# riffusion/riffusion-hobby

Measured on AMD Instinct MI355X. Metric: spectrogram_tiles_per_sec_griffinlim32, higher is better.
Workload: dtype f32

## Files before the change

riffusion-hobby_amd/csrc/rfx_imel.hip:

```cpp
#include <hip/hip_runtime.h>

#include "rfx_core.h"
#include "rfx_kernels.h"
#include <stdlib.h>

namespace rfx {

constexpr int kImelThreads = 256;

template <int BPT>
__global__ void __launch_bounds__(kImelThreads) imel_kernel(ImelArgs a) {
  extern __shared__ __attribute__((aligned(16))) char smem[];
  const ImelTables& tb = a.tb;
  const int nb = tb.f_hi - tb.f_lo;
  float* spec_s = reinterpret_cast<float*>(smem);
  float* w_s = spec_s + ((nb + 3) & ~3);
  float* diff_s = w_s + ((tb.nnz + 3) & ~3);
  float* red_s = diff_s + ((a.M + 1 + 3) & ~3);
  float* hist_s = red_s + 4;

  const int frame = blockIdx.x;
  const int b = frame / a.T, t = frame - b * a.T;
  const int clip = b / a.C;
  const int tid = threadIdx.x;
// ... 160 lines not shown
    for (int p4 = tid; p4 < (a.out_stride >> 2); p4 += nthr) {
      const int4 b = pb4[p4];
      out4[p4] = float4{value_at(b.x), value_at(b.y), value_at(b.z), value_at(b.w)};
    }
  } else {
    for (int p = tid; p < a.out_stride; p += nthr) out[p] = value_at(tb.pos_bin[p]);
  }
}

constexpr float kImelScale = 8.673617379884035e-19f;
constexpr float kImelUnscale = 1152921504606846976.0f;
__device__ __forceinline__ void imel_set_scale(ImelArgs& a, int clip) {
  a.sc = a.clip_scale ? a.clip_scale[2 * clip] : kImelScale;
  a.un = a.clip_scale ? a.clip_scale[2 * clip + 1] : kImelUnscale;
}
#ifndef RFX_IMEL_CLAMP
#define RFX_IMEL_CLAMP 1
#endif
#ifndef RFX_IMEL_UFORM
#define RFX_IMEL_UFORM 1
#endif

__device__ __forceinline__ float clamp_step(float x) {
#if RFX_IMEL_CLAMP
  return __builtin_amdgcn_fmed3f(x, 0.f, 1.f);
#else
  return fmaxf(0.f, x);
#endif
}

#ifndef RFX_IMEL_PK
#define RFX_IMEL_PK 1
#endif
#if RFX_IMEL_PK
using c2 = float __attribute__((ext_vector_type(2)));
__device__ __forceinline__ c2 bc2(float x) { return c2{x, x}; }
__device__ __forceinline__ c2 pk_step_clamp(c2 spec, unsigned long long nl2, c2 buf) {
#if RFX_IMEL_CLAMP
  asm("v_pk_fma_f32 %0, %1, %2, %0 clamp" : "+v"(spec) : "s"(nl2), "v"(buf));
  return spec;
#else
  const float nl = __builtin_bit_cast(float, (unsigned)nl2);
  const c2 r = __builtin_elementwise_fma(bc2(nl), buf, spec);
  return c2{fmaxf(0.f, r.x), fmaxf(0.f, r.y)};
#endif
}

template <int N, bool UF>
struct GroupState {
  static constexpr int NP = (N + 1) / 2;
  c2 spec[NP], buf[NP], w0[NP], w1[NP];
  int f0, n;
};

template <int N, bool UF>
__device__ __forceinline__ void group_load(GroupState<N, UF>& g, int grp, const ImelArgs& a, int frame, unsigned rbase, float scale) {
  const ImelTables& tb = a.tb;
  g.f0 = grp >= 0 ? tb.grp_start[grp] : 0;
  g.n = grp >= 0 ? tb.grp_start[grp + 1] - g.f0 : 0;
#pragma unroll
  for (int i = 0; i < 2 * g.NP; ++i) {
    const bool ok = i < g.n;
    const int f = g.f0 + (ok ? i : 0);
    const float w0 = ok ? tb.bin_w0[f] : 0.f, w1 = ok ? tb.bin_w1[f] : 0.f;
    const float sp = ok ? scale * (a.spec0 ? a.spec0[(size_t)frame * a.n_stft + f] : rand_unit(rbase, f)) : 0.f;
    if (i & 1) { g.w0[i >> 1].y = w0; g.w1[i >> 1].y = w1; g.spec[i >> 1].y = sp; g.buf[i >> 1].y = 0.f; }
    else       { g.w0[i >> 1].x = w0; g.w1[i >> 1].x = w1; g.spec[i >> 1].x = sp; g.buf[i >> 1].x = 0.f; }
  }
}
template <int N, bool UF>
__device__ __forceinline__ void group_ab(const GroupState<N, UF>& g, float& A, float& B) {
  c2 sa = bc2(0.f), sb = bc2(0.f);
#pragma unroll
  for (int i = 0; i < g.NP; ++i) {
    sa = __builtin_elementwise_fma(g.w0[i], g.spec[i], sa);
    sb = __builtin_elementwise_fma(g.w1[i], g.spec[i], sb);
  }
  A = sa.x + sa.y;
  B = sb.x + sb.y;
}
template <int N, bool UF>
__device__ __forceinline__ void group_step(GroupState<N, UF>& g, float d0, float d1, float mom, unsigned long long nl2) {
  const c2 vm = bc2(mom), v0 = bc2(d0), v1 = bc2(d1), vd = bc2(d0 - d1);
#pragma unroll
  for (int i = 0; i < g.NP; ++i) {
    c2 bnew;
    if (UF) {
      bnew = __builtin_elementwise_fma(vm, g.buf[i], v1);
      bnew = __builtin_elementwise_fma(vd, g.w0[i], bnew);
    } else {
      bnew = vm * g.buf[i];
      bnew = __builtin_elementwise_fma(v0, g.w0[i], bnew);
      bnew = __builtin_elementwise_fma(v1, g.w1[i], bnew);
    }
    g.buf[i] = bnew;
  }
#pragma unroll
  for (int i = 0; i < g.NP; ++i) g.spec[i] = pk_step_clamp(g.spec[i], nl2, g.buf[i]);
}
template <int N, bool UF>
__device__ __forceinline__ void group_stage(const GroupState<N, UF>& g, const ImelTables& tb, float* stage, float unscale) {
#pragma unroll
  for (int i = 0; i < 2 * g.NP; ++i)
    if (i < g.n) stage[g.f0 + i - tb.f_lo] = unscale * ((i & 1) ? g.spec[i >> 1].y : g.spec[i >> 1].x);
}
#else
template <int N, bool UF>
struct GroupState {
  float spec[N], buf[N], w0[N], w1[N];
  int f0, n;
};

template <int N, bool UF>
__device__ __forceinline__ void group_load(GroupState<N, UF>& g, int grp, const ImelArgs& a, int frame, unsigned rbase, float scale) {
  const ImelTables& tb = a.tb;
  g.f0 = grp >= 0 ? tb.grp_start[grp] : 0;
  g.n = grp >= 0 ? tb.grp_start[grp + 1] - g.f0 : 0;
#pragma unroll
  for (int i = 0; i < N; ++i) {
    const bool ok = i < g.n;
    const int f = g.f0 + (ok ? i : 0);
    g.w0[i] = ok ? tb.bin_w0[f] : 0.f;
    g.w1[i] = ok ? tb.bin_w1[f] : 0.f;
    g.spec[i] = ok ? scale * (a.spec0 ? a.spec0[(size_t)frame * a.n_stft + f] : rand_unit(rbase, f)) : 0.f;
    g.buf[i] = 0.f;
  }
}
template <int N, bool UF>
__device__ __forceinline__ void group_ab(const GroupState<N, UF>& g, float& A, float& B) {
  float a0 = 0.f, a1 = 0.f, b0 = 0.f, b1 = 0.f;
#pragma unroll
  for (int i = 0; i < N; i += 2) {
    a0 = fmaf(g.w0[i], g.spec[i], a0);
    b0 = fmaf(g.w1[i], g.spec[i], b0);
    if (i + 1 < N) {
      a1 = fmaf(g.w0[i + 1], g.spec[i + 1], a1);
      b1 = fmaf(g.w1[i + 1], g.spec[i + 1], b1);
    }
  }
  A = a0 + a1;
  B = b0 + b1;
}
template <int N, bool UF>
__device__ __forceinline__ void group_step(GroupState<N, UF>& g, float d0, float d1, float mom, unsigned long long nl2) {
  const float lrg = -__builtin_bit_cast(float, (unsigned)nl2);
  const float dd = d0 - d1;
#pragma unroll
  for (int i = 0; i < N; ++i) {
    float bnew;
    if (UF) {
      bnew = fmaf(mom, g.buf[i], d1);
      bnew = fmaf(dd, g.w0[i], bnew);
    } else {
      bnew = mom * g.buf[i];
      bnew = fmaf(d0, g.w0[i], bnew);
      bnew = fmaf(d1, g.w1[i], bnew);
    }
    g.buf[i] = bnew;
    g.spec[i] = clamp_step(fmaf(-lrg, bnew, g.spec[i]));
  }
}
template <int N, bool UF>
__device__ __forceinline__ void group_stage(const GroupState<N, UF>& g, const ImelTables& tb, float* stage, float unscale) {
#pragma unroll
  for (int i = 0; i < N; ++i)
    if (i < g.n) stage[g.f0 + i - tb.f_lo] = unscale * g.spec[i];
}

#endif

template <int NLO, int NHI, bool UF>
__device__ __forceinline__ void imel_group_body(ImelArgs a, char* smem, int tid, int frame, bool live) {
  const ImelTables& tb = a.tb;
  const int M = a.M;
  float* Ab = reinterpret_cast<float*>(smem);
  float* Bb = Ab + 2 * (M + 4);
  float* part = Bb + 2 * (M + 4);

  const int b = frame / a.T, t = frame - b * a.T;
  const int clip = b / a.C;
  const int steps = a.it_limit ? a.it_limit[clip] : a.max_iter;
  if (a.it_limit && steps >= a.max_iter) return;
  const unsigned rbase = rand_frame_key(a.seed, a.frame_base + (unsigned long long)frame);
  imel_set_scale(a, clip);

  const int gH = (M - 1 - tid >= 0) ? M - 1 - tid : -1;
  const int gL = (tid < M - kImelThreads) ? tid : -1;
  const float kScale = RFX_IMEL_CLAMP ? a.sc : 1.f, kUnscale = RFX_IMEL_CLAMP ? a.un : 1.f;
  GroupState<NLO, false> lo;
  GroupState<NHI, UF> hi;
  group_load(lo, gL, a, frame, rbase, kScale);
  group_load(hi, gH, a, frame, rbase, kScale);
  auto melat = [&](int m) { return (m >= 0 && m < M) ? kScale * a.mel[((size_t)b * M + m) * a.T + t] : 0.f; };
  const float mL0 = gL >= 0 ? melat(gL) : 0.f, mL1 = gL >= 0 ? melat(gL + 1) : 0.f;
  const float mH0 = gH >= 0 ? melat(gH) : 0.f, mH1 = gH >= 0 ? melat(gH + 1) : 0.f;
  for (int i = tid; i < 4 * (M + 4); i += kImelThreads) Ab[i] = 0.f;
  const float lrg = a.lr * (-2.0f / (float)(a.C * a.T));
  const unsigned nlb = __builtin_amdgcn_readfirstlane(__builtin_bit_cast(unsigned, -lrg));
  const unsigned long long nl2 = ((unsigned long long)nlb << 32) | nlb;
  const int xL = (gL >= 0 ? gL : M + 1) + 1, xH = (gH >= 0 ? gH : M + 1) + 1;
  const bool noH1 = UF && gH == M - 1;
  const int wave = tid >> 6;
  __syncthreads();

  auto sgd_step = [&](int it, float* __restrict__ Ap, float* __restrict__ Bp) {
    float AL, BL, AH, BH;
    group_ab(lo, AL, BL);
    group_ab(hi, AH, BH);
    Ap[xL] = AL; Bp[xL] = BL;
    Ap[xH] = AH; Bp[xH] = BH;
    __syncthreads();
    const float bLm = Bp[xL - 1], aLp = Ap[xL + 1], bHm = Bp[xH - 1], aHp = Ap[xH + 1];
    const float dL0 = mL0 - AL - bLm;
    const float dL1 = mL1 - aLp - BL;
    const float dH0 = mH0 - AH - bHm;
    const float dH1 = noH1 ? 0.f : mH1 - aHp - BH;
#ifndef RFX_ABL_IMEL_NO_LOSS
    const float uL = kUnscale * dL0, uH = kUnscale * dH0;
    const float sq = wave_sum(fmaf(uL, uL, uH * uH));
    if ((tid & 63) == 0) part[4 * it + wave] = sq;
#endif
    group_step(lo, dL0, dL1, a.momentum, nl2);
    group_step(hi, dH0, dH1, a.momentum, nl2);
  };
  float* const A0 = Ab, * const A1 = Ab + (M + 4), * const B0 = Bb, * const B1 = Bb + (M + 4);
  int it = 0;
  for (; it + 1 < steps; it += 2) {
    sgd_step(it, A0, B0);
    sgd_step(it + 1, A1, B1);
  }
  if (it < steps) sgd_step(it, A0, B0);
  __syncthreads();

  float* stage = reinterpret_cast<float*>(smem + imel_group_lds_bytes(M, a.max_iter));
  group_stage(lo, tb, stage, kUnscale);
  group_stage(hi, tb, stage, kUnscale);
  __syncthreads();
  if (!live) return;
  imel_emit_frame(a, stage, frame, rbase, tid, kImelThreads);
  if (a.loss_hist && !a.it_limit)
    for (int i = tid; i < a.max_iter; i += kImelThreads)
      a.loss_hist[(size_t)frame * a.max_iter + i] = i < steps ? (part[4 * i] + part[4 * i + 1]) + (part[4 * i + 2] + part[4 * i + 3]) : 0.f;
}

template <int NLO, int NHI>
__global__ void __launch_bounds__(kImelThreads) imel_group_kernel(ImelArgs a) {
  extern __shared__ __attribute__((aligned(16))) char smem[];
  imel_group_body<NLO, NHI, false>(a, smem, threadIdx.x, blockIdx.x, true);
}
#ifndef RFX_IMEL_WAVES_PER_EU
#define RFX_IMEL_WAVES_PER_EU 4
#endif
#ifndef RFX_IMEL_WAVES_PER_EU_UF
#define RFX_IMEL_WAVES_PER_EU_UF 4
#endif
#ifndef RFX_IMEL_FPW
#define RFX_IMEL_FPW 1
#endif

template <int FPW, int WPE, bool UF, int L0, int H0, int L1, int H1, int L2, int H2, int L3, int H3>
__global__ void __launch_bounds__(kImelThreads * FPW) __attribute__((amdgpu_waves_per_eu(WPE)))
imel_group_kernel_perwave(ImelArgs a) {
  extern __shared__ __attribute__((aligned(16))) char smem[];
  const int wave = __builtin_amdgcn_readfirstlane(threadIdx.x >> 6);
  const int slot = wave >> 2, w4 = wave & 3;
  const int cls = FPW == 1 ? w4 : FPW == 2 ? (slot ? 3 - w4 : w4) : ((w4 + slot) & 3);
  const int tid = cls * 64 + (threadIdx.x & 63);
  const int nframes = a.B * a.T;
  int frame = blockIdx.x * FPW + slot;
  const bool live = frame < nframes;
  if (!live) frame = nframes - 1;
  char* my = smem + (size_t)slot * imel_frame_lds_bytes(a.M, a.max_iter, a.tb.f_hi - a.tb.f_lo);
  switch (cls) {
    case 0: imel_group_body<L0, H0, UF>(a, my, tid, frame, live); break;
    case 1: imel_group_body<L1, H1, UF>(a, my, tid, frame, live); break;
    case 2: imel_group_body<L2, H2, UF>(a, my, tid, frame, live); break;
    default: imel_group_body<L3, H3, UF>(a, my, tid, frame, live); break;
  }
}


#if RFX_IMEL_PK
constexpr int kDppWaveShl1 = 0x130, kDppWaveShr1 = 0x138;
template <int CTRL>
__device__ __forceinline__ float wave_shift(float old, float src) {
  return __builtin_bit_cast(float, __builtin_amdgcn_update_dpp(__builtin_bit_cast(int, old), __builtin_bit_cast(int, src), CTRL, 0xf, 0xf, false));
}
__device__ __forceinline__ c2 pk_add_clamp(c2 x, c2 v) {
  asm("v_pk_add_f32 %0, %0, %1 clamp" : "+v"(x) : "v"(v));
  return x;
}
__device__ __forceinline__ c2 pk_fma_clamp(c2 x, c2 v, c2 m) {
  asm("v_pk_fma_f32 %0, %1, %2, %0 clamp" : "+v"(x) : "v"(v), "v"(m));
  return x;
}

__device__ __forceinline__ void fma_in_place(float& x, unsigned m_sgpr, float c) { asm("v_fma_f32 %0, %1, %0, %2" : "+v"(x) : "s"(m_sgpr), "v"(c)); }

template <int NP, int NF, bool UF>
struct WvChunk {
  static constexpr int NT = NP - NF;
  c2 spec[NP];
  c2 mask[NT > 0 ? NT : 1];
  float a0, s0, a1, s1;
  float m0;
  float C, G;
};

template <int NP, int NF, bool UF>
__device__ __forceinline__ void wv_load(WvChunk<NP, NF, UF>& k, int g, const ImelArgs& a, int frame, int b, int t, unsigned rbase) {
  const ImelTables& tb = a.tb;
  const int f0 = tb.grp_start[g], n = tb.grp_start[g + 1] - f0;
  k.a0 = tb.lin[g];
  k.s0 = tb.lin[a.M + g];
  k.a1 = tb.lin[2 * a.M + g];
  k.s1 = tb.lin[3 * a.M + g];
  k.m0 = a.sc * a.mel[((size_t)b * a.M + g) * a.T + t];
  k.C = 0.f;
  k.G = 0.f;
#pragma unroll
  for (int i = 0; i < 2 * NP; ++i) {
    const bool ok = i < n;
    const int f = f0 + (ok ? i : 0);
    const float sp = ok ? a.sc * (a.spec0 ? a.spec0[(size_t)frame * a.n_stft + f] : rand_unit(rbase, f)) : 0.f;
    if (i & 1) k.spec[i >> 1].y = sp; else k.spec[i >> 1].x = sp;
    if (i >= 2 * NF) {
      if (i & 1) k.mask[(i >> 1) - NF].y = ok ? 1.f : 0.f; else k.mask[(i >> 1) - NF].x = ok ? 1.f : 0.f;
    }
  }
}
template <int NPA, int NFA, int NPB, int NFB, bool UFA, bool UFB>
__device__ __forceinline__ void wv_sums2(const WvChunk<NPA, NFA, UFA>& ka, const WvChunk<NPB, NFB, UFB>& kb, c2& SA, c2& QA, c2& SB, c2& QB) {
  static_assert(NPA >= 2 && NPB >= 2, "every chunk holds at least two pairs");
  SA = ka.spec[0] + ka.spec[1];
  SB = kb.spec[0] + kb.spec[1];
  QA = ka.spec[1];
  QB = kb.spec[1];
#pragma unroll
  for (int p = 2; p < (NPA > NPB ? NPA : NPB); ++p) {
    if (p < NPA) SA = SA + ka.spec[p];
    if (p < NPB) SB = SB + kb.spec[p];
    if (p < NPA) QA = __builtin_elementwise_fma(bc2((float)p), ka.spec[p], QA);
    if (p < NPB) QB = __builtin_elementwise_fma(bc2((float)p), kb.spec[p], QB);
  }
}
template <int NP, int NF, bool UF>
__device__ __forceinline__ void wv_update(WvChunk<NP, NF, UF>& k, float vx, float vy, float w2) {
  const c2 base = c2{vx, vy}, s2 = bc2(w2);
  c2 v[NP];
  v[0] = base;
#pragma unroll
  for (int p = 1; p < NP; ++p) v[p] = __builtin_elementwise_fma(bc2((float)p), s2, base);
#pragma unroll
  for (int p = 0; p < NP; ++p) k.spec[p] = p < NF ? pk_add_clamp(k.spec[p], v[p]) : pk_fma_clamp(k.spec[p], v[p], k.mask[p < NF ? 0 : p - NF]);
}
template <int NP, int NF, bool UF>
__device__ __forceinline__ void wv_stage(const WvChunk<NP, NF, UF>& k, int g, const ImelTables& tb, float* stage, float unscale) {
  const int f0 = tb.grp_start[g], n = tb.grp_start[g + 1] - f0;
#pragma unroll
  for (int i = 0; i < 2 * NP; ++i)
    if (i < n) stage[f0 + i - tb.f_lo] = unscale * ((i & 1) ? k.spec[i >> 1].y : k.spec[i >> 1].x);
}

template <int NP, bool UF>
struct LineGroup {
  c2 spec[NP], mask[NP];
  float a0, s0, a1, s1;
  float C, G;
};
template <int NP, bool UF>
__device__ __forceinline__ void line_load(LineGroup<NP, UF>& k, int g, const ImelArgs& a, int frame, unsigned rbase) {
  const ImelTables& tb = a.tb;
  const int f0 = g >= 0 ? tb.grp_start[g] : 0, n = g >= 0 ? tb.grp_start[g + 1] - f0 : 0;
  k.a0 = g >= 0 ? tb.lin[g] : 0.f;
  k.s0 = g >= 0 ? tb.lin[a.M + g] : 0.f;
  k.a1 = g >= 0 ? tb.lin[2 * a.M + g] : 0.f;
  k.s1 = g >= 0 ? tb.lin[3 * a.M + g] : 0.f;
  k.C = 0.f;
  k.G = 0.f;
#pragma unroll
  for (int i = 0; i < 2 * NP; ++i) {
    const bool ok = i < n;
    const int f = f0 + (ok ? i : 0);
    const float sp = ok ? a.sc * (a.spec0 ? a.spec0[(size_t)frame * a.n_stft + f] : rand_unit(rbase, f)) : 0.f;
    if (i & 1) { k.spec[i >> 1].y = sp; k.mask[i >> 1].y = ok ? 1.f : 0.f; }
    else       { k.spec[i >> 1].x = sp; k.mask[i >> 1].x = ok ? 1.f : 0.f; }
  }
}
template <int NP, bool UF>
__device__ __forceinline__ void line_ab(const LineGroup<NP, UF>& k, float& A, float& B) {
  static_assert(NP >= 2, "a line group holds at least two pairs");
  c2 Sa = k.spec[0], Sb = k.spec[1], Qa = bc2(0.f), Qb = k.spec[1];
#pragma unroll
  for (int p = 2; p < NP; ++p) {
    if (p & 1) { Sb = Sb + k.spec[p]; Qb = __builtin_elementwise_fma(bc2((float)p), k.spec[p], Qb); }
    else       { Sa = Sa + k.spec[p]; Qa = __builtin_elementwise_fma(bc2((float)p), k.spec[p], Qa); }
  }
  const c2 S = Sa + Sb, Q = Qa + Qb;
  const float s = S.x + S.y, h = Q.x + Q.y;
  const float q = fmaf(2.f, h, S.y);
  A = fmaf(k.s0, q, k.a0 * s);
  B = UF ? s - A : fmaf(k.s1, q, k.a1 * s);
}
template <int NP, bool UF>
__device__ __forceinline__ void line_step(LineGroup<NP, UF>& k, float n0, float n1, float mom) {
  float cc, st;
  if (UF) {
    const float dd = n0 - n1;
    cc = fmaf(dd, k.a0, n1);
    st = dd * k.s0;
  } else {
    cc = fmaf(n1, k.a1, n0 * k.a0);
    st = fmaf(n1, k.s1, n0 * k.s0);
  }
  k.C = fmaf(mom, k.C, cc);
  k.G = fmaf(mom, k.G, st);
  const c2 base = c2{k.C, k.C + k.G}, s2 = bc2(k.G + k.G);
#pragma unroll
  for (int p = 0; p < NP; ++p) {
    const c2 v = p == 0 ? base : __builtin_elementwise_fma(bc2((float)p), s2, base);
    k.spec[p] = pk_fma_clamp(k.spec[p], v, k.mask[p]);
  }
}
template <int NP, bool UF>
__device__ __forceinline__ void line_stage(const LineGroup<NP, UF>& k, int g, const ImelTables& tb, float* stage, float unscale) {
  if (g < 0) return;
  const int f0 = tb.grp_start[g], n = tb.grp_start[g + 1] - f0;
#pragma unroll
  for (int i = 0; i < 2 * NP; ++i)
    if (i < n) stage[f0 + i - tb.f_lo] = unscale * ((i & 1) ? k.spec[i >> 1].y : k.spec[i >> 1].x);
}

template <int NLO, int NHI, bool UF>
__device__ __forceinline__ void imel_line_body(ImelArgs a, char* smem, int tid, int frame) {
  const ImelTables& tb = a.tb;
  const int M = a.M;
  float* Ab = reinterpret_cast<float*>(smem);
  float* Bb = Ab + 2 * (M + 4);
  float* part = Bb + 2 * (M + 4);
  const int b = frame / a.T, t = frame - b * a.T;
  const int clip = b / a.C;
  const int steps = a.it_limit ? a.it_limit[clip] : a.max_iter;
  if (a.it_limit && steps >= a.max_iter) return;
  const unsigned rbase = rand_frame_key(a.seed, a.frame_base + (unsigned long long)frame);
  imel_set_scale(a, clip);
  int gH = (M - 1 - tid >= 0) ? M - 1 - tid : -1;
  int gL = (tid < M - kImelThreads) ? tid : -1;
  if (gH >= 0 && gH < tb.line_from) {
    gL = gH;
    gH = -1;
  }
  GroupState<NLO, false> lo;
  LineGroup<(NHI + 1) / 2, UF> hi;
  group_load(lo, gL, a, frame, rbase, a.sc);
  line_load(hi, gH, a, frame, rbase);
  auto melat = [&](int m) { return (m >= 0 && m < M) ? a.sc * a.mel[((size_t)b * M + m) * a.T + t] : 0.f; };
  const float mL0 = gL >= 0 ? melat(gL) : 0.f, mL1 = gL >= 0 ? melat(gL + 1) : 0.f;
  const float mH0 = gH >= 0 ? melat(gH) : 0.f, mH1 = gH >= 0 ? melat(gH + 1) : 0.f;
  for (int i = tid; i < 4 * (M + 4); i += kImelThreads) Ab[i] = 0.f;
  const float lrg = a.lr * (-2.0f / (float)(a.C * a.T));
  const float nl = -lrg;
  const unsigned nlb = __builtin_amdgcn_readfirstlane(__builtin_bit_cast(unsigned, nl));
  const unsigned long long nl2 = ((unsigned long long)nlb << 32) | nlb;
  const int xL = (gL >= 0 ? gL : M + 1) + 1, xH = (gH >= 0 ? gH : M + 1) + 1;
  const bool noH1 = UF && gH == M - 1;
  const int wave = tid >> 6;
  __syncthreads();

  auto sgd_step = [&](int it, float* __restrict__ Ap, float* __restrict__ Bp) {
    float AL, BL, AH, BH;
    group_ab(lo, AL, BL);
    line_ab(hi, AH, BH);
    Ap[xL] = AL; Bp[xL] = BL;
    Ap[xH] = AH; Bp[xH] = BH;
    __syncthreads();
    const float bLm = Bp[xL - 1], aLp = Ap[xL + 1], bHm = Bp[xH - 1], aHp = Ap[xH + 1];
    const float dL0 = mL0 - AL - bLm;
    const float dL1 = mL1 - aLp - BL;
    const float dH0 = mH0 - AH - bHm;
    const float dH1 = noH1 ? 0.f : mH1 - aHp - BH;
    const float uL = a.un * dL0, uH = a.un * dH0;
    const float sq = wave_sum(fmaf(uL, uL, uH * uH));
    if ((tid & 63) == 0) part[4 * it + wave] = sq;
    group_step(lo, dL0, dL1, a.momentum, nl2);
    line_step(hi, nl * dH0, nl * dH1, a.momentum);
  };
  float* const A0 = Ab, * const A1 = Ab + (M + 4), * const B0 = Bb, * const B1 = Bb + (M + 4);
  int it = 0;
  for (; it + 1 < steps; it += 2) {
    sgd_step(it, A0, B0);
    sgd_step(it + 1, A1, B1);
  }
  if (it < steps) sgd_step(it, A0, B0);
  __syncthreads();

  float* stage = reinterpret_cast<float*>(smem + imel_group_lds_bytes(M, a.max_iter));
  group_stage(lo, tb, stage, a.un);
  line_stage(hi, gH, tb, stage, a.un);
  __syncthreads();
  imel_emit_frame(a, stage, frame, rbase, tid, kImelThreads);
  if (a.loss_hist && !a.it_limit)
    for (int i = tid; i < a.max_iter; i += kImelThreads)
      a.loss_hist[(size_t)frame * a.max_iter + i] = i < steps ? (part[4 * i] + part[4 * i + 1]) + (part[4 * i + 2] + part[4 * i + 3]) : 0.f;
}

template <bool UF, int L0, int H0, int L1, int H1, int L2, int H2, int L3, int H3>
__global__ void __launch_bounds__(kImelThreads) __attribute__((amdgpu_waves_per_eu(2, 2))) imel_line_kernel_perwave(ImelArgs a) {
  extern __shared__ __attribute__((aligned(16))) char smem[];
  const int cls = __builtin_amdgcn_readfirstlane(threadIdx.x >> 6);
  const int tid = threadIdx.x;
  const int frame = blockIdx.x;
  switch (cls) {
    case 0: imel_line_body<L0, H0, UF>(a, smem, tid, frame); break;
    case 1: imel_line_body<L1, H1, UF>(a, smem, tid, frame); break;
    case 2: imel_line_body<L2, H2, UF>(a, smem, tid, frame); break;
    default: imel_line_body<L3, H3, UF>(a, smem, tid, frame); break;
  }
}

#define RFX_WV_CHUNKS(X) X(0) X(1) X(2) X(3) X(4) X(5) X(6) X(7)
#define RFX_WV_LO(X) X(0) X(1) X(2) X(3)
#define RFX_WV_HI(X) X(4) X(5) X(6) X(7)

template <bool UFH>
__global__ void __launch_bounds__(64) __attribute__((amdgpu_waves_per_eu(2, 2))) imel_wave_kernel(ImelArgs a) {
  extern __shared__ __attribute__((aligned(16))) char smem[];
  float* part = reinterpret_cast<float*>(smem);
  const ImelTables& tb = a.tb;
  const int lane = threadIdx.x, frame = blockIdx.x;
  const int b = frame / a.T, t = frame - b * a.T;
  const int clip = b / a.C;
  const int steps = a.it_limit ? a.it_limit[clip] : a.max_iter;
  if (a.it_limit && steps >= a.max_iter) return;
  const unsigned rbase = rand_frame_key(a.seed, a.frame_base + (unsigned long long)frame);
  imel_set_scale(a, clip);
  for (int i = lane; i < a.max_iter; i += 64) part[i] = 0.f;
  const unsigned part_lds = (unsigned)(size_t)(__attribute__((address_space(3))) char*)smem;

#define RFX_WV_DECL(c, UF) WvChunk<kImelWavePairs[c], kImelWaveFullPairs[c], UF> k##c;
  RFX_WV_DECL(0, false) RFX_WV_DECL(1, false) RFX_WV_DECL(2, false) RFX_WV_DECL(3, false)
  RFX_WV_DECL(4, UFH) RFX_WV_DECL(5, UFH) RFX_WV_DECL(6, UFH) RFX_WV_DECL(7, UFH)
#undef RFX_WV_DECL
#define RFX_WV_LOAD(c) wv_load(k##c, imel_wave_group(c, lane), a, frame, b, t, rbase);
  RFX_WV_CHUNKS(RFX_WV_LOAD)
#undef RFX_WV_LOAD

  const float nl = -(a.lr * (-2.0f / (float)(a.C * a.T)));
  const unsigned mom_s = __builtin_amdgcn_readfirstlane(__builtin_bit_cast(unsigned, a.momentum));
  __builtin_amdgcn_s_waitcnt(0xc07f);

  for (int it = 0; it < steps; ++it) {
    float A0, A1, A2, A3, A4, A5, A6, A7, B0, B1, B2, B3, B4, B5, B6, B7;
    {
      c2 S0, Q0, S1, Q1, S2, Q2, S3, Q3;
      wv_sums2(k0, k1, S0, Q0, S1, Q1);
      wv_sums2(k2, k3, S2, Q2, S3, Q3);
#define RFX_WV_T1(c) const float s##c = S##c.x + S##c.y, h##c = Q##c.x + Q##c.y;
#define RFX_WV_T2(c) const float q##c = fmaf(2.f, h##c, S##c.y), e##c = k##c.a0 * s##c, g##c = k##c.a1 * s##c;
#define RFX_WV_T3(c) A##c = fmaf(k##c.s0, q##c, e##c); B##c = fmaf(k##c.s1, q##c, g##c);
      RFX_WV_LO(RFX_WV_T1) RFX_WV_LO(RFX_WV_T2) RFX_WV_LO(RFX_WV_T3)
#undef RFX_WV_T2
#undef RFX_WV_T3
    }
    {
      c2 S4, Q4, S5, Q5, S6, Q6, S7, Q7;
      wv_sums2(k4, k5, S4, Q4, S5, Q5);
      wv_sums2(k6, k7, S6, Q6, S7, Q7);
#define RFX_WV_T2(c) const float q##c = fmaf(2.f, h##c, S##c.y), e##c = k##c.a0 * s##c;
#define RFX_WV_T3(c) A##c = fmaf(k##c.s0, q##c, e##c);
#define RFX_WV_T4(c) B##c = UFH ? s##c - A##c : fmaf(k##c.s1, q##c, k##c.a1 * s##c);
      RFX_WV_HI(RFX_WV_T1) RFX_WV_HI(RFX_WV_T2) RFX_WV_HI(RFX_WV_T3) RFX_WV_HI(RFX_WV_T4)
#undef RFX_WV_T1
#undef RFX_WV_T2
#undef RFX_WV_T3
#undef RFX_WV_T4
    }
#define RFX_WV_R1(c) const float r##c = k##c.m0 - A##c;
    RFX_WV_CHUNKS(RFX_WV_R1)
#undef RFX_WV_R1
    const float p0 = wave_shift<kDppWaveShr1>(0.f, B0), p1 = wave_shift<kDppWaveShl1>(B0, B1), p2 = wave_shift<kDppWaveShr1>(B1, B2),
                p3 = wave_shift<kDppWaveShl1>(B2, B3), p4 = wave_shift<kDppWaveShr1>(B3, B4), p5 = wave_shift<kDppWaveShl1>(B4, B5),
                p6 = wave_shift<kDppWaveShr1>(B5, B6), p7 = wave_shift<kDppWaveShl1>(B6, B7);
#define RFX_WV_R2(c) const float d0##c = r##c - p##c;
    RFX_WV_CHUNKS(RFX_WV_R2)
#undef RFX_WV_R2
#ifndef RFX_ABL_IMEL_NO_LOSS
    {
#define RFX_WV_L1(c) const float u##c = a.un * d0##c;
      RFX_WV_CHUNKS(RFX_WV_L1)
#undef RFX_WV_L1
      const float sqa = fmaf(u6, u6, fmaf(u4, u4, fmaf(u2, u2, u0 * u0))), sqb = fmaf(u7, u7, fmaf(u5, u5, fmaf(u3, u3, u1 * u1)));
      asm volatile("ds_add_f32 %0, %1" ::"v"(part_lds + 4u * (unsigned)it), "v"(sqa + sqb) : "memory");
    }
#endif
#define RFX_WV_N0(c) const float n0##c = nl * d0##c;
    RFX_WV_CHUNKS(RFX_WV_N0)
#undef RFX_WV_N0
    const float n10 = wave_shift<kDppWaveShl1>(n01, n00), n11 = wave_shift<kDppWaveShr1>(n02, n01), n12 = wave_shift<kDppWaveShl1>(n03, n02),
                n13 = wave_shift<kDppWaveShr1>(n04, n03), n14 = wave_shift<kDppWaveShl1>(n05, n04), n15 = wave_shift<kDppWaveShr1>(n06, n05),
                n16 = wave_shift<kDppWaveShl1>(n07, n06), n17 = wave_shift<kDppWaveShr1>(0.f, n07);
    const float dd4 = n04 - n14, dd5 = n05 - n15, dd6 = n06 - n16, dd7 = n07 - n17;
    const float x0 = n00 * k0.a0, x1 = n01 * k1.a0, x2 = n02 * k2.a0, x3 = n03 * k3.a0;
    const float y0 = n00 * k0.s0, y1 = n01 * k1.s0, y2 = n02 * k2.s0, y3 = n03 * k3.s0;
    const float cc0 = fmaf(n10, k0.a1, x0), cc1 = fmaf(n11, k1.a1, x1), cc2 = fmaf(n12, k2.a1, x2), cc3 = fmaf(n13, k3.a1, x3);
    const float st0 = fmaf(n10, k0.s1, y0), st1 = fmaf(n11, k1.s1, y1), st2 = fmaf(n12, k2.s1, y2), st3 = fmaf(n13, k3.s1, y3);
#define RFX_WV_G0(c) const float cc##c = UFH ? fmaf(dd##c, k##c.a0, n1##c) : fmaf(n1##c, k##c.a1, n0##c * k##c.a0), \
                                 st##c = UFH ? dd##c * k##c.s0 : fmaf(n1##c, k##c.s1, n0##c * k##c.s0);
    RFX_WV_HI(RFX_WV_G0)
#undef RFX_WV_G0
#define RFX_WV_G1(c) fma_in_place(k##c.C, mom_s, cc##c); fma_in_place(k##c.G, mom_s, st##c);
#define RFX_WV_G3(c) const float vx##c = k##c.C, vy##c = k##c.C + k##c.G, w2##c = k##c.G + k##c.G;
    RFX_WV_CHUNKS(RFX_WV_G1) RFX_WV_CHUNKS(RFX_WV_G3)
#undef RFX_WV_G1
#undef RFX_WV_G3
#define RFX_WV_UPDATE(c) wv_update(k##c, vx##c, vy##c, w2##c);
    RFX_WV_CHUNKS(RFX_WV_UPDATE)
#undef RFX_WV_UPDATE
  }

  float* stage = part + a.max_iter;
#define RFX_WV_STAGE(c) wv_stage(k##c, imel_wave_group(c, lane), tb, stage, a.un);
  RFX_WV_CHUNKS(RFX_WV_STAGE)
#undef RFX_WV_STAGE
  __builtin_amdgcn_fence(__ATOMIC_RELEASE, "wavefront");
  __builtin_amdgcn_wave_barrier();
  __builtin_amdgcn_fence(__ATOMIC_ACQUIRE, "wavefront");
  imel_emit_frame(a, stage, frame, rbase, lane, 64);
  if (a.loss_hist && !a.it_limit) {
    __builtin_amdgcn_s_waitcnt(0xc07f);
    for (int i = lane; i < a.max_iter; i += 64) a.loss_hist[(size_t)frame * a.max_iter + i] = i < steps ? part[i] : 0.f;
  }
}
#undef RFX_WV_CHUNKS
#undef RFX_WV_LO
#undef RFX_WV_HI
#endif

__global__ void __launch_bounds__(1024) imel_scan_kernel(const float* __restrict__ loss_hist, int* __restrict__ it_stop,
                                                        int* __restrict__ any_early, int nclips, int C, int T, int max_iter,
                                                        float tol_loss, float tol_change) {
  extern __shared__ float scan_smem[];
  float* part = scan_smem;
  float* mean = scan_smem + 1024;
  const int clip = blockIdx.x;
  if (clip >= nclips) return;
  const int nframes = C * T;
  const int i = threadIdx.x & 255, g = threadIdx.x >> 8;
  const float* base = loss_hist + (size_t)clip * nframes * max_iter;
  for (int it0 = 0; it0 < max_iter; it0 += 256) {
    const int it = it0 + i;
    float s0 = 0.f, s1 = 0.f;
    if (it < max_iter) {
      int f = g;
      for (; f + 4 < nframes; f += 8) {
        s0 += base[(size_t)f * max_iter + it];
        s1 += base[(size_t)(f + 4) * max_iter + it];
      }
      if (f < nframes) s0 += base[(size_t)f * max_iter + it];
    }
    part[g * 256 + i] = s0 + s1;
    __syncthreads();
    if (g == 0 && it < max_iter) mean[it] = ((part[i] + part[256 + i]) + (part[512 + i] + part[768 + i])) / (float)nframes;
    __syncthreads();
  }
  if (threadIdx.x == 0) {
    float prev = __builtin_inff();
    int stop = max_iter;
    for (int it = 0; it < max_iter; ++it) {
      const float loss = mean[it];
      if (loss < tol_loss || fabsf(prev - loss) < tol_change) { stop = it + 1; break; }
      prev = loss;
    }
    it_stop[clip] = stop;
    if (stop < max_iter) atomicExch(any_early, 1);
  }
}

template <int FPW, int SET, bool UF>
static void launch_perwave(const ImelArgs& a, hipStream_t stream) {
  const int nframes = a.B * a.T;
  const size_t lds = FPW * imel_frame_lds_bytes(a.M, a.max_iter, a.tb.f_hi - a.tb.f_lo);
  constexpr const int* lo = SET == 0 ? kImelLoCap : kImelLoCapWide;
  constexpr const int* hi = SET == 0 ? kImelHiCap : kImelHiCapWide;
  constexpr int wpe = SET == 0 ? (UF ? RFX_IMEL_WAVES_PER_EU_UF : RFX_IMEL_WAVES_PER_EU) : 3;
  hipLaunchKernelGGL((imel_group_kernel_perwave<FPW, wpe, UF, lo[0], hi[0], lo[1], hi[1], lo[2], hi[2], lo[3], hi[3]>), dim3((nframes + FPW - 1) / FPW),
                     dim3(kImelThreads * FPW), lds, stream, a);
}

int imel_kernel_choice(const ImelTables& tb, int M, int max_iter, int variant) {
  const int band = tb.f_hi - tb.f_lo;
  constexpr size_t kPlainLds = 64 * 1024;
#if RFX_IMEL_PK && RFX_IMEL_WAVE
  if (tb.wave_ok && variant == 0 && sizeof(float) * ((size_t)max_iter + (size_t)band) <= kPlainLds) return 4;
#endif
  const size_t frame_lds = imel_frame_lds_bytes(M, max_iter, band);
#if RFX_IMEL_PK
  if (tb.fast_ok == 5 && variant == 0 && frame_lds <= kPlainLds) return 5;
#endif
  if (tb.fast_ok && tb.fast_ok != 5 && variant != 2 && !(variant == 1 && tb.fast_ok == 3) && frame_lds <= kPlainLds) {
    if (tb.fast_ok == 2 && variant != 1) return 2;
    if (tb.fast_ok == 3 && variant != 1) return 3;
    return 1;
  }
  return 0;
}

hipError_t launch_imel(const ImelArgs& a, int variant, hipStream_t stream) {
  const int choice = imel_kernel_choice(a.tb, a.M, a.max_iter, variant);
#if RFX_IMEL_PK && RFX_IMEL_WAVE
  if (choice == 4) {
    const size_t lds = sizeof(float) * ((size_t)a.max_iter + (size_t)(a.tb.f_hi - a.tb.f_lo));
    if (a.tb.unit_form) hipLaunchKernelGGL(imel_wave_kernel<true>, dim3(a.B * a.T), dim3(64), lds, stream, a);
    else hipLaunchKernelGGL(imel_wave_kernel<false>, dim3(a.B * a.T), dim3(64), lds, stream, a);
    return hipGetLastError();
  }
#endif
#if RFX_IMEL_PK
  if (choice == 5) {
    constexpr const int* lo = kImelLoCapLine;
    constexpr const int* hi = kImelHiCapLine;
    const size_t lds = imel_frame_lds_bytes(a.M, a.max_iter, a.tb.f_hi - a.tb.f_lo);
    if (a.tb.unit_form) hipLaunchKernelGGL((imel_line_kernel_perwave<true, lo[0], hi[0], lo[1], hi[1], lo[2], hi[2], lo[3], hi[3]>), dim3(a.B * a.T), dim3(kImelThreads), lds, stream, a);
    else hipLaunchKernelGGL((imel_line_kernel_perwave<false, lo[0], hi[0], lo[1], hi[1], lo[2], hi[2], lo[3], hi[3]>), dim3(a.B * a.T), dim3(kImelThreads), lds, stream, a);
    return hipGetLastError();
  }
#endif
  if (choice >= 1 && choice <= 3) {
    const bool fixup = a.it_limit != nullptr;
    if (choice == 2) {
      if (a.tb.unit_form && RFX_IMEL_UFORM) {
        if (fixup) launch_perwave<1, 0, true>(a, stream); else launch_perwave<RFX_IMEL_FPW, 0, true>(a, stream);
      } else {
        if (fixup) launch_perwave<1, 0, false>(a, stream); else launch_perwave<RFX_IMEL_FPW, 0, false>(a, stream);
      }
    } else if (choice == 3) {
      if (a.tb.unit_form && RFX_IMEL_UFORM) {
        if (fixup) launch_perwave<1, 1, true>(a, stream); else launch_perwave<RFX_IMEL_FPW, 1, true>(a, stream);
      } else {
        if (fixup) launch_perwave<1, 1, false>(a, stream); else launch_perwave<RFX_IMEL_FPW, 1, false>(a, stream);
      }
    } else {
      hipLaunchKernelGGL((imel_group_kernel<8, 24>), dim3(a.B * a.T), dim3(kImelThreads), imel_frame_lds_bytes(a.M, a.max_iter, a.tb.f_hi - a.tb.f_lo), stream, a);
    }
    return hipGetLastError();
  }
  const int nb = a.tb.f_hi - a.tb.f_lo;
  const size_t lds = sizeof(float) * (((nb + 3) & ~3) + ((a.tb.nnz + 3) & ~3) + ((a.M + 1 + 3) & ~3) + 4 + a.max_iter);
  const int bpt = (nb + kImelThreads - 1) / kImelThreads;
  if (bpt <= 16) {
    (void)hipFuncSetAttribute((const void*)imel_kernel<16>, hipFuncAttributeMaxDynamicSharedMemorySize, (int)lds);
    hipLaunchKernelGGL(imel_kernel<16>, dim3(a.B * a.T), dim3(kImelThreads), lds, stream, a);
  } else {
    (void)hipFuncSetAttribute((const void*)imel_kernel<36>, hipFuncAttributeMaxDynamicSharedMemorySize, (int)lds);
    hipLaunchKernelGGL(imel_kernel<36>, dim3(a.B * a.T), dim3(kImelThreads), lds, stream, a);
  }
  return hipGetLastError();
}

__device__ __forceinline__ float wave_max(float x) {
#pragma unroll
  for (int off = 32; off > 0; off >>= 1) x = fmaxf(x, __shfl_xor(x, off, 64));
  return x;
}
__global__ void __launch_bounds__(256) range_max_kernel(const float* __restrict__ x, size_t count, unsigned* __restrict__ keys) {
  const float* p = x + (size_t)blockIdx.y * count;
  float mx = 0.f;
  for (size_t i = (size_t)blockIdx.x * 256 + threadIdx.x; i < count; i += (size_t)gridDim.x * 256) mx = fmaxf(mx, fabsf(p[i]));
  mx = wave_max(mx);
  if ((threadIdx.x & 63) == 0 && mx > 0.f) atomicMax(&keys[blockIdx.y], __float_as_uint(mx));
}
__global__ void __launch_bounds__(64) range_finish_kernel(const unsigned* __restrict__ keys, int groups, float hint, float* __restrict__ imel_scale,
                                                          float* __restrict__ gl_scale, int rows, int mel_units) {
  const int g = blockIdx.x * 64 + threadIdx.x;
  if (g >= groups) return;
  const float mx = hint > 0.f ? hint : __uint_as_float(keys[g]);
  int k = 0;
  if (mx > 0.f) {
    if (mx < __builtin_inff()) (void)frexpf(mx, &k);
    else k = 129;
  }
  int e, j;
  range_exponents(k, mel_units, &e, &j);
  if (imel_scale) {
    imel_scale[2 * g] = ldexpf(1.f, -e);
    imel_scale[2 * g + 1] = ldexpf(1.f, e);
  }
  if (gl_scale) {
    const float eps2 = fmaxf(ldexpf(1e-32f, -2 * j), 1.17549435e-38f);
    for (int r = 0; r < rows; ++r) {
      gl_scale[2 * ((size_t)g * rows + r)] = ldexpf(1.f, -j);
      gl_scale[2 * ((size_t)g * rows + r) + 1] = eps2;
    }
  }
}
hipError_t launch_range_scale(const float* x, size_t count, int groups, float hint, unsigned* keys, float* imel_scale, float* gl_scale, int rows,
                              int mel_units, hipStream_t stream) {
  if (!(hint > 0.f)) {
    hipError_t e = hipMemsetAsync(keys, 0, sizeof(unsigned) * (size_t)groups, stream);
    if (e != hipSuccess) return e;
    size_t chunks = (count + 256 * 64 - 1) / (256 * 64);
    if (chunks > 256) chunks = 256;
    if (chunks < 1) chunks = 1;
    for (int g0 = 0; g0 < groups; g0 += 65535) {
      const int n = groups - g0 < 65535 ? groups - g0 : 65535;
      hipLaunchKernelGGL(range_max_kernel, dim3((unsigned)chunks, (unsigned)n), dim3(256), 0, stream, x + (size_t)g0 * count, count, keys + g0);
      if ((e = hipGetLastError()) != hipSuccess) return e;
    }
  }
  hipLaunchKernelGGL(range_finish_kernel, dim3((groups + 63) / 64), dim3(64), 0, stream, keys, groups, hint, imel_scale, gl_scale, rows, mel_units);
  return hipGetLastError();
}

hipError_t launch_imel_scan(const float* loss_hist, int* it_stop, int* any_early, int nclips, int C, int T, int max_iter,
                            float tol_loss, float tol_change, hipStream_t stream) {
  hipLaunchKernelGGL(imel_scan_kernel, dim3(nclips), dim3(1024), sizeof(float) * (1024 + (size_t)max_iter), stream, loss_hist, it_stop, any_early, nclips, C, T,
                     max_iter, tol_loss, tol_change);
  return hipGetLastError();
}

}
```

Measured before the change: 2147.

## Pack per-chunk line coefficients into float pairs and vectorize wave update math

Moves the per-group line coefficients and mel targets out of each chunk into paired c2 structs, so that neighbouring chunks are processed together with packed (v_pk) FMA/mul instructions. Scalar residual, loss and gradient arithmetic is rewritten in pairs, with a v_pk_mov gather feeding the DPP shifts. The update step also folds the 2*G scaling into the constants so fewer intermediate values are needed. The aim is to cut VALU instruction count in the hot iteration loop. Packed ops and the contract(off) pragma could change register pressure and scheduling, and the inline asm limits what the compiler can optimize.

```diff
diff --git a/riffusion-hobby_amd/csrc/rfx_imel.hip b/riffusion-hobby_amd/csrc/rfx_imel.hip
--- a/riffusion-hobby_amd/csrc/rfx_imel.hip
+++ b/riffusion-hobby_amd/csrc/rfx_imel.hip
@@ -486,20 +486,13 @@
   static constexpr int NT = NP - NF;
   c2 spec[NP];
   c2 mask[NT > 0 ? NT : 1];
-  float a0, s0, a1, s1;
-  float m0;
   float C, G;
 };
 
 template <int NP, int NF, bool UF>
-__device__ __forceinline__ void wv_load(WvChunk<NP, NF, UF>& k, int g, const ImelArgs& a, int frame, int b, int t, unsigned rbase) {
+__device__ __forceinline__ void wv_load(WvChunk<NP, NF, UF>& k, int g, const ImelArgs& a, int frame, unsigned rbase) {
   const ImelTables& tb = a.tb;
   const int f0 = tb.grp_start[g], n = tb.grp_start[g + 1] - f0;
-  k.a0 = tb.lin[g];
-  k.s0 = tb.lin[a.M + g];
-  k.a1 = tb.lin[2 * a.M + g];
-  k.s1 = tb.lin[3 * a.M + g];
-  k.m0 = a.sc * a.mel[((size_t)b * a.M + g) * a.T + t];
   k.C = 0.f;
   k.G = 0.f;
 #pragma unroll
@@ -529,14 +522,42 @@
   }
 }
 template <int NP, int NF, bool UF>
-__device__ __forceinline__ void wv_update(WvChunk<NP, NF, UF>& k, float vx, float vy, float w2) {
-  const c2 base = c2{vx, vy}, s2 = bc2(w2);
+__device__ __forceinline__ void wv_update(WvChunk<NP, NF, UF>& k, float vy) {
+  const c2 base = c2{k.C, vy}, g2 = bc2(k.G);
   c2 v[NP];
   v[0] = base;
 #pragma unroll
-  for (int p = 1; p < NP; ++p) v[p] = __builtin_elementwise_fma(bc2((float)p), s2, base);
+  for (int p = 1; p < NP; ++p) v[p] = __builtin_elementwise_fma(bc2((float)(2 * p)), g2, base);
 #pragma unroll
   for (int p = 0; p < NP; ++p) k.spec[p] = p < NF ? pk_add_clamp(k.spec[p], v[p]) : pk_fma_clamp(k.spec[p], v[p], k.mask[p < NF ? 0 : p - NF]);
+}
+__device__ __forceinline__ float wv_add(float x, float y) {
+  float s;
+  asm("v_add_f32 %0, %1, %2" : "=v"(s) : "v"(x), "v"(y));
+  return s;
+}
+__device__ __forceinline__ float wv_fma2(float h, float y) {
+  float q;
+  asm("v_fma_f32 %0, 2.0, %1, %2" : "=v"(q) : "v"(h), "v"(y));
+  return q;
+}
+__device__ __forceinline__ c2 wv_gather(c2 x, c2 y) {
+  c2 r;
+  asm("v_pk_mov_b32 %0, %1, %2 op_sel:[1,0]" : "=v"(r) : "v"(x), "v"(y));
+  return r;
+}
+struct WvLines {
+  c2 a0, s0, a1, s1;
+  c2 m0;
+};
+__device__ __forceinline__ void wv_load_lines(WvLines& l, int c, int lane, const ImelArgs& a, int b, int t) {
+  const ImelTables& tb = a.tb;
+  const int g0 = imel_wave_group(c, lane), g1 = imel_wave_group(c + 1, lane);
+  l.a0 = c2{tb.lin[g0], tb.lin[g1]};
+  l.s0 = c2{tb.lin[a.M + g0], tb.lin[a.M + g1]};
+  l.a1 = c2{tb.lin[2 * a.M + g0], tb.lin[2 * a.M + g1]};
+  l.s1 = c2{tb.lin[3 * a.M + g0], tb.lin[3 * a.M + g1]};
+  l.m0 = c2{a.sc * a.mel[((size_t)b * a.M + g0) * a.T + t], a.sc * a.mel[((size_t)b * a.M + g1) * a.T + t]};
 }
 template <int NP, int NF, bool UF>
 __device__ __forceinline__ void wv_stage(const WvChunk<NP, NF, UF>& k, int g, const ImelTables& tb, float* stage, float unscale) {
@@ -703,8 +724,6 @@
 }
 
 #define RFX_WV_CHUNKS(X) X(0) X(1) X(2) X(3) X(4) X(5) X(6) X(7)
-#define RFX_WV_LO(X) X(0) X(1) X(2) X(3)
-#define RFX_WV_HI(X) X(4) X(5) X(6) X(7)
 
 template <bool UFH>
 __global__ void __launch_bounds__(64) __attribute__((amdgpu_waves_per_eu(2, 2))) imel_wave_kernel(ImelArgs a) {
@@ -725,81 +744,77 @@
   RFX_WV_DECL(0, false) RFX_WV_DECL(1, false) RFX_WV_DECL(2, false) RFX_WV_DECL(3, false)
   RFX_WV_DECL(4, UFH) RFX_WV_DECL(5, UFH) RFX_WV_DECL(6, UFH) RFX_WV_DECL(7, UFH)
 #undef RFX_WV_DECL
-#define RFX_WV_LOAD(c) wv_load(k##c, imel_wave_group(c, lane), a, frame, b, t, rbase);
+#define RFX_WV_LOAD(c) wv_load(k##c, imel_wave_group(c, lane), a, frame, rbase);
   RFX_WV_CHUNKS(RFX_WV_LOAD)
 #undef RFX_WV_LOAD
+  WvLines l0, l1, l2, l3;
+  wv_load_lines(l0, 0, lane, a, b, t);
+  wv_load_lines(l1, 2, lane, a, b, t);
+  wv_load_lines(l2, 4, lane, a, b, t);
+  wv_load_lines(l3, 6, lane, a, b, t);
 
   const float nl = -(a.lr * (-2.0f / (float)(a.C * a.T)));
   const unsigned mom_s = __builtin_amdgcn_readfirstlane(__builtin_bit_cast(unsigned, a.momentum));
   __builtin_amdgcn_s_waitcnt(0xc07f);
 
   for (int it = 0; it < steps; ++it) {
-    float A0, A1, A2, A3, A4, A5, A6, A7, B0, B1, B2, B3, B4, B5, B6, B7;
+#pragma clang fp contract(off)
+    c2 sP01, sP23, sP45, sP67, qP01, qP23, qP45, qP67;
     {
-      c2 S0, Q0, S1, Q1, S2, Q2, S3, Q3;
+      c2 S0, Q0, S1, Q1, S2, Q2, S3, Q3, S4, Q4, S5, Q5, S6, Q6, S7, Q7;
       wv_sums2(k0, k1, S0, Q0, S1, Q1);
       wv_sums2(k2, k3, S2, Q2, S3, Q3);
-#define RFX_WV_T1(c) const float s##c = S##c.x + S##c.y, h##c = Q##c.x + Q##c.y;
-#define RFX_WV_T2(c) const float q##c = fmaf(2.f, h##c, S##c.y), e##c = k##c.a0 * s##c, g##c = k##c.a1 * s##c;
-#define RFX_WV_T3(c) A##c = fmaf(k##c.s0, q##c, e##c); B##c = fmaf(k##c.s1, q##c, g##c);
-      RFX_WV_LO(RFX_WV_T1) RFX_WV_LO(RFX_WV_T2) RFX_WV_LO(RFX_WV_T3)
-#undef RFX_WV_T2
-#undef RFX_WV_T3
-    }
-    {
-      c2 S4, Q4, S5, Q5, S6, Q6, S7, Q7;
       wv_sums2(k4, k5, S4, Q4, S5, Q5);
       wv_sums2(k6, k7, S6, Q6, S7, Q7);
-#define RFX_WV_T2(c) const float q##c = fmaf(2.f, h##c, S##c.y), e##c = k##c.a0 * s##c;
-#define RFX_WV_T3(c) A##c = fmaf(k##c.s0, q##c, e##c);
-#define RFX_WV_T4(c) B##c = UFH ? s##c - A##c : fmaf(k##c.s1, q##c, k##c.a1 * s##c);
-      RFX_WV_HI(RFX_WV_T1) RFX_WV_HI(RFX_WV_T2) RFX_WV_HI(RFX_WV_T3) RFX_WV_HI(RFX_WV_T4)
-#undef RFX_WV_T1
-#undef RFX_WV_T2
-#undef RFX_WV_T3
-#undef RFX_WV_T4
-    }
-#define RFX_WV_R1(c) const float r##c = k##c.m0 - A##c;
-    RFX_WV_CHUNKS(RFX_WV_R1)
-#undef RFX_WV_R1
-    const float p0 = wave_shift<kDppWaveShr1>(0.f, B0), p1 = wave_shift<kDppWaveShl1>(B0, B1), p2 = wave_shift<kDppWaveShr1>(B1, B2),
-                p3 = wave_shift<kDppWaveShl1>(B2, B3), p4 = wave_shift<kDppWaveShr1>(B3, B4), p5 = wave_shift<kDppWaveShl1>(B4, B5),
-                p6 = wave_shift<kDppWaveShr1>(B5, B6), p7 = wave_shift<kDppWaveShl1>(B6, B7);
-#define RFX_WV_R2(c) const float d0##c = r##c - p##c;
-    RFX_WV_CHUNKS(RFX_WV_R2)
-#undef RFX_WV_R2
+#define RFX_WV_T(c0, c1) sP##c0##c1 = c2{wv_add(S##c0.x, S##c0.y), wv_add(S##c1.x, S##c1.y)}; \
+      qP##c0##c1 = c2{wv_fma2(Q##c0.x + Q##c0.y, S##c0.y), wv_fma2(Q##c1.x + Q##c1.y, S##c1.y)};
+      RFX_WV_T(0, 1) RFX_WV_T(2, 3) RFX_WV_T(4, 5) RFX_WV_T(6, 7)
+#undef RFX_WV_T
+    }
+    const c2 A01 = __builtin_elementwise_fma(l0.s0, qP01, l0.a0 * sP01), A23 = __builtin_elementwise_fma(l1.s0, qP23, l1.a0 * sP23),
+             A45 = __builtin_elementwise_fma(l2.s0, qP45, l2.a0 * sP45), A67 = __builtin_elementwise_fma(l3.s0, qP67, l3.a0 * sP67);
+    const c2 B01 = __builtin_elementwise_fma(l0.s1, qP01, l0.a1 * sP01), B23 = __builtin_elementwise_fma(l1.s1, qP23, l1.a1 * sP23);
+    const c2 B45 = UFH ? sP45 - A45 : __builtin_elementwise_fma(l2.s1, qP45, l2.a1 * sP45);
+    const c2 B67 = UFH ? sP67 - A67 : __builtin_elementwise_fma(l3.s1, qP67, l3.a1 * sP67);
+    const c2 r01 = l0.m0 - A01, r23 = l1.m0 - A23, r45 = l2.m0 - A45, r67 = l3.m0 - A67;
+    const c2 d01 = c2{r01.x - wave_shift<kDppWaveShr1>(0.f, B01.x), r01.y - wave_shift<kDppWaveShl1>(B01.x, B01.y)},
+             d23 = c2{r23.x - wave_shift<kDppWaveShr1>(B01.y, B23.x), r23.y - wave_shift<kDppWaveShl1>(B23.x, B23.y)},
+             d45 = c2{r45.x - wave_shift<kDppWaveShr1>(B23.y, B45.x), r45.y - wave_shift<kDppWaveShl1>(B45.x, B45.y)},
+             d67 = c2{r67.x - wave_shift<kDppWaveShr1>(B45.y, B67.x), r67.y - wave_shift<kDppWaveShl1>(B67.x, B67.y)};
 #ifndef RFX_ABL_IMEL_NO_LOSS
     {
-#define RFX_WV_L1(c) const float u##c = a.un * d0##c;
-      RFX_WV_CHUNKS(RFX_WV_L1)
-#undef RFX_WV_L1
-      const float sqa = fmaf(u6, u6, fmaf(u4, u4, fmaf(u2, u2, u0 * u0))), sqb = fmaf(u7, u7, fmaf(u5, u5, fmaf(u3, u3, u1 * u1)));
-      asm volatile("ds_add_f32 %0, %1" ::"v"(part_lds + 4u * (unsigned)it), "v"(sqa + sqb) : "memory");
-    }
-#endif
-#define RFX_WV_N0(c) const float n0##c = nl * d0##c;
-    RFX_WV_CHUNKS(RFX_WV_N0)
-#undef RFX_WV_N0
-    const float n10 = wave_shift<kDppWaveShl1>(n01, n00), n11 = wave_shift<kDppWaveShr1>(n02, n01), n12 = wave_shift<kDppWaveShl1>(n03, n02),
-                n13 = wave_shift<kDppWaveShr1>(n04, n03), n14 = wave_shift<kDppWaveShl1>(n05, n04), n15 = wave_shift<kDppWaveShr1>(n06, n05),
-                n16 = wave_shift<kDppWaveShl1>(n07, n06), n17 = wave_shift<kDppWaveShr1>(0.f, n07);
-    const float dd4 = n04 - n14, dd5 = n05 - n15, dd6 = n06 - n16, dd7 = n07 - n17;
-    const float x0 = n00 * k0.a0, x1 = n01 * k1.a0, x2 = n02 * k2.a0, x3 = n03 * k3.a0;
-    const float y0 = n00 * k0.s0, y1 = n01 * k1.s0, y2 = n02 * k2.s0, y3 = n03 * k3.s0;
-    const float cc0 = fmaf(n10, k0.a1, x0), cc1 = fmaf(n11, k1.a1, x1), cc2 = fmaf(n12, k2.a1, x2), cc3 = fmaf(n13, k3.a1, x3);
-    const float st0 = fmaf(n10, k0.s1, y0), st1 = fmaf(n11, k1.s1, y1), st2 = fmaf(n12, k2.s1, y2), st3 = fmaf(n13, k3.s1, y3);
-#define RFX_WV_G0(c) const float cc##c = UFH ? fmaf(dd##c, k##c.a0, n1##c) : fmaf(n1##c, k##c.a1, n0##c * k##c.a0), \
-                                 st##c = UFH ? dd##c * k##c.s0 : fmaf(n1##c, k##c.s1, n0##c * k##c.s0);
-    RFX_WV_HI(RFX_WV_G0)
-#undef RFX_WV_G0
-#define RFX_WV_G1(c) fma_in_place(k##c.C, mom_s, cc##c); fma_in_place(k##c.G, mom_s, st##c);
-#define RFX_WV_G3(c) const float vx##c = k##c.C, vy##c = k##c.C + k##c.G, w2##c = k##c.G + k##c.G;
-    RFX_WV_CHUNKS(RFX_WV_G1) RFX_WV_CHUNKS(RFX_WV_G3)
-#undef RFX_WV_G1
-#undef RFX_WV_G3
-#define RFX_WV_UPDATE(c) wv_update(k##c, vx##c, vy##c, w2##c);
-    RFX_WV_CHUNKS(RFX_WV_UPDATE)
-#undef RFX_WV_UPDATE
+      const c2 un2 = bc2(a.un);
+      const c2 u01 = un2 * d01, u23 = un2 * d23, u45 = un2 * d45, u67 = un2 * d67;
+      const c2 sq = __builtin_elementwise_fma(u67, u67, __builtin_elementwise_fma(u45, u45, __builtin_elementwise_fma(u23, u23, u01 * u01)));
+      asm volatile("ds_add_f32 %0, %1" ::"v"(part_lds + 4u * (unsigned)it), "v"(sq.x + sq.y) : "memory");
+    }
+#endif
+    const c2 nl2 = bc2(nl);
+    const c2 n001 = nl2 * d01, n023 = nl2 * d23, n045 = nl2 * d45, n067 = nl2 * d67;
+    const c2 o01 = wv_gather(n001, n023), o23 = wv_gather(n023, n045), o45 = wv_gather(n045, n067), o67 = wv_gather(n067, bc2(0.f));
+    const c2 n101 = c2{wave_shift<kDppWaveShl1>(o01.x, n001.x), wave_shift<kDppWaveShr1>(o01.y, n001.y)},
+             n123 = c2{wave_shift<kDppWaveShl1>(o23.x, n023.x), wave_shift<kDppWaveShr1>(o23.y, n023.y)},
+             n145 = c2{wave_shift<kDppWaveShl1>(o45.x, n045.x), wave_shift<kDppWaveShr1>(o45.y, n045.y)},
+             n167 = c2{wave_shift<kDppWaveShl1>(o67.x, n067.x), wave_shift<kDppWaveShr1>(o67.y, n067.y)};
+    const c2 cc01 = __builtin_elementwise_fma(n101, l0.a1, n001 * l0.a0), st01 = __builtin_elementwise_fma(n101, l0.s1, n001 * l0.s0);
+    const c2 cc23 = __builtin_elementwise_fma(n123, l1.a1, n023 * l1.a0), st23 = __builtin_elementwise_fma(n123, l1.s1, n023 * l1.s0);
+    c2 cc45, st45, cc67, st67;
+    if (UFH) {
+      const c2 dd45 = __builtin_elementwise_fma(nl2, d45, -n145), dd67 = __builtin_elementwise_fma(nl2, d67, -n167);
+      cc45 = __builtin_elementwise_fma(dd45, l2.a0, n145);
+      st45 = dd45 * l2.s0;
+      cc67 = __builtin_elementwise_fma(dd67, l3.a0, n167);
+      st67 = dd67 * l3.s0;
+    } else {
+      cc45 = __builtin_elementwise_fma(n145, l2.a1, n045 * l2.a0);
+      st45 = __builtin_elementwise_fma(n145, l2.s1, n045 * l2.s0);
+      cc67 = __builtin_elementwise_fma(n167, l3.a1, n067 * l3.a0);
+      st67 = __builtin_elementwise_fma(n167, l3.s1, n067 * l3.s0);
+    }
+#define RFX_WV_G(c, cc, st) fma_in_place(k##c.C, mom_s, cc); fma_in_place(k##c.G, mom_s, st); wv_update(k##c, k##c.C + k##c.G);
+    RFX_WV_G(0, cc01.x, st01.x) RFX_WV_G(1, cc01.y, st01.y) RFX_WV_G(2, cc23.x, st23.x) RFX_WV_G(3, cc23.y, st23.y)
+    RFX_WV_G(4, cc45.x, st45.x) RFX_WV_G(5, cc45.y, st45.y) RFX_WV_G(6, cc67.x, st67.x) RFX_WV_G(7, cc67.y, st67.y)
+#undef RFX_WV_G
   }
 
   float* stage = part + a.max_iter;
@@ -816,8 +831,6 @@
   }
 }
 #undef RFX_WV_CHUNKS
-#undef RFX_WV_LO
-#undef RFX_WV_HI
 #endif
 
 __global__ void __launch_bounds__(1024) imel_scan_kernel(const float* __restrict__ loss_hist, int* __restrict__ it_stop,
```

After: 2185 (median of 6 runs). +1.8%, better.
